# vineetbansal/scarlet

Measured on AMD Instinct MI355X. Metric: PGM iters/sec on 10k 5-band 64x64 scenes, higher is better.
Workload: dtype f32

## Files before the change

scarlet_amd/csrc/fused2.h:

```cpp
#pragma once
#include "fused.h"

#define SC_FB2 512
#define SC_NW2 (SC_FB2 / SC_WAVE)
#define SC_PAIR_VEC_FLOATS 512
__host__ __device__ inline size_t fused2_lds_bytes(int K, int H, int W)
{
    return sizeof(float) * ((size_t)K * H * tile_stride(W) + (size_t)K * SC_PAIR_VEC_FLOATS);
}
__host__ __device__ inline size_t fused2_exact_lds_bytes(int KM, int XS)
{
    return sizeof(float) * ((size_t)KM * XS * SC_XS_STRIDE + (size_t)KM * SC_PAIR_VEC_FLOATS);
}

struct KsLengths {
    unsigned short v[2][32];
    static constexpr int fast_len(int n)
    {
        for (int m = n;; ++m) {
            int q = m;
            while (q % 2 == 0) q /= 2;
            while (q % 3 == 0) q /= 3;
            while (q % 5 == 0) q /= 5;
            if (q == 1) return m;
        }
    }
    constexpr KsLengths() : v{}
    {
        for (int r = 0; r < 32; ++r) {
            const int F = fast_len(2 * (2 * r + 1) + 10);
            int Fe = F;
            while (Fe & 1) Fe = fast_len(Fe + 1);
            v[0][r] = (unsigned short)F; v[1][r] = (unsigned short)Fe;
        }
    }
};
__device__ const KsLengths sc_ks_lengths = KsLengths();
__device__ __forceinline__ unsigned ks_request_lengths(int tid)
{
    return tid < 64 ? (unsigned)(&sc_ks_lengths.v[0][0])[tid] : 0u;
}
__device__ __forceinline__ void ks_fill_lengths(unsigned short (*fl)[32], int tid, unsigned requested)
{
    if (tid < 64) (&fl[0][0])[tid] = (unsigned short)requested;
}
__device__ __forceinline__ KsGeom ks_geom(const SymWindow &s, const unsigned short (*fl)[32])
{
    KsGeom g;
    g.h = s.h; g.w = s.w; g.ry = s.h / 2; g.rx = s.w / 2;
    g.ntr = round16(s.h) >> 4; g.wp = round16(s.w); g.ntc = g.wp >> 4;
    g.Fy = uniform((int)fl[0][g.ry]);
    g.Fx = uniform((int)fl[1][g.rx]);
    return g;
}

template <int KM, int BM, int XS, bool P>
__device__ __forceinline__ int iterate2_body(const FusedArgs &a, const int s, const int c0, const int it_old, const bool resident,
                                             const bool reentered = false)
{
    static_assert(KM <= 4, "one pair of waves per component");
    static_assert(1 + KM * BM <= 32 && 4 * SC_NW2 == 32, "the partial sums are combined by 32 rows of 16 lanes");
    constexpr bool X = XS > 0;
    extern __shared__ __align__(16) float lds[];
    const int K = X ? KM : a.K, B = X ? BM : a.B, H = X ? XS : a.H, W = X ? XS : a.W, HW = H * W, LW = X ? SC_XS_STRIDE : tile_stride(W);
    const int tile_floats = H * LW;
#ifndef SC_TILE_B128
#define SC_TILE_B128 1
#endif
    auto tl4 = [](const float *p) {
        if constexpr (X && SC_TILE_B128 && (SC_XS_STRIDE % 4) == 0) return *reinterpret_cast<const float4 *>(p);
        else return lds_load4(p);
    };
    auto ts4 = [](float *p, float4 v) {
        if constexpr (X && SC_TILE_B128 && (SC_XS_STRIDE % 4) == 0) *reinterpret_cast<float4 *>(p) = v;
        else lds_store4(p, v);
    };
    const bool symmetric = X ? true : a.symmetric != 0, monotonic = X ? true : a.monotonic != 0;
    float *tiles = lds;
    float *vecs = lds + (size_t)K * tile_floats;
    constexpr int NG = KM * (KM + 1) / 2;
    constexpr int NP = 1 + KM * BM;
    constexpr int GPT = 2;
    constexpr int GPW = 8;
    __shared__ float red[4 * SC_NW2][NP > NG ? NP : NG];
    __shared__ double mat[2][KM * KM > BM * BM ? KM * KM : BM * BM];
    __shared__ float sed_s[KM * BM], sed_new[KM * BM];
    __shared__ float step_s[2];
    __shared__ double conv_s[KM][2], conv_m[KM][2][2];
    __shared__ int lstop_s[KM];
    __shared__ float nmax_s[KM][2];
    __shared__ int pair_flag[KM][2];
    __shared__ int arrive_s;
    __shared__ double cent_s[KM][2][3];
    __shared__ unsigned short fl_s[2][32];
    __shared__ int ctl_s[2][2];
    __shared__ int carry_cen[KM][2];
    __shared__ double carry_sh[KM][2];
    __shared__ float carry_sed[KM * BM];
    __shared__ short rowrange_s[KM][2][2];
    __shared__ unsigned place_s;
    const int tid = threadIdx.x, lane = tid & 63, wid = uniform(tid >> 6);
    float *const morph0 = a.morph[0], *const morph1 = a.morph[1], *const sed0 = a.sed[0], *const sed1 = a.sed[1];
    const float *min_g = (c0 ? morph1 : morph0) + (size_t)s * K * HW;
    float *mout_g = (c0 ? morph0 : morph1) + (size_t)s * K * HW;
    const float *sed_in = (c0 ? sed1 : sed0) + (size_t)s * K * B;
    float *sed_out = (c0 ? sed0 : sed1) + (size_t)s * K * B;
    const int it_new = it_old + 1;
    const int ngroups = HW >> 2, gpr = W >> 2;
    const float *img = a.images + (size_t)s * B * HW;
    const float *wgt = (!X && a.weights) ? a.weights + (size_t)s * B * HW : nullptr;
#define STAMP(i) do { if (a.stamps && tid == 0) a.stamps[(size_t)s * 16 + (i)] = (long long)__builtin_amdgcn_s_memtime(); } while (0)
#ifdef SC_STAMP_WORKER
#define WSTAMP(i) do { if (a.stamps && lane == 0) a.stamps[(size_t)s * 16 + 12 + (i)] = (long long)__builtin_amdgcn_s_memtime(); } while (0)
#else
#define WSTAMP(i) do { } while (0)
#endif
#ifdef SC_STAMP_PAIRS
    long long pst[3] = {0, 0, 0};
#define PSTAMP(i) do { if (a.stamps) pst[i] = (long long)__builtin_amdgcn_s_memtime(); } while (0)
#else
#define PSTAMP(i) do { } while (0)
#endif
    STAMP(0);
    if (a.stamps && tid == 0) a.stamps[(size_t)s * 16 + 7] = (long long)__builtin_amdgcn_s_memrealtime();
#ifdef SC_STAMP_PERIOD
    if (P && a.stamps && tid == 0) a.stamps[(size_t)a.S * 16 + (size_t)s * 2 + (it_new & 1)] = (long long)__builtin_amdgcn_s_memrealtime();
#endif
    if (P && a.stamps && tid == 0 && !reentered) {
        a.stamps[(size_t)s * 16 + 14] = (long long)__builtin_amdgcn_s_memrealtime();
        a.stamps[(size_t)s * 16 + 15] = (long long)__builtin_amdgcn_s_getreg(4 | (0 << 6) | (31 << 11))
                                        | ((long long)__builtin_amdgcn_s_getreg(20 | (0 << 6) | (31 << 11)) << 32);
    }
    const unsigned fl_req = ks_request_lengths(tid);
    const int n_present = a.ncomp ? scene_ncomp(a.ncomp, s, K) : K;
    const int slot = wid >> 1;
    int kp = slot;
    if constexpr (X) {
        unsigned place = 0x03020100u;
        if (P) { const unsigned lp = place_s; if (reentered) place = (unsigned)uniform((int)lp); }
        if (!(P && reentered) && !a.no_place) {
            int cost[KM];
#pragma unroll
            for (int j = 0; j < KM; ++j) {
                const int ccy = uniform(a.centers[2 * (s * K + j)]), ccx = uniform(a.centers[2 * (s * K + j) + 1]);
                const SymWindow w = sym_window(H, W, ccy, ccx);
                const int ntr = round16(w.h) >> 4, ntc = round16(w.w) >> 4;
                cost[j] = (j < n_present && !w.centered) ? ntr * ntc * (ntr + ntc) : 0;
            }
            place = 0;
#pragma unroll
            for (int j = 0; j < KM; ++j) {
                int rank = 0;
#pragma unroll
                for (int i = 0; i < KM; ++i) rank += (cost[i] > cost[j] || (cost[i] == cost[j] && i < j)) ? 1 : 0;
                place |= (unsigned)j << (8 * (rank ^ (rank >> 1)));
            }
        }
        if (P && !reentered && tid == 0) place_s = place;
        kp = (int)((place >> (8 * slot)) & (KM - 1));
    }
    int pre_cy = 0, pre_cx = 0;
    double pre_dy = 0, pre_dx = 0;
    if (X && kp < K) {
        const int cpre = s * K + kp;
        if (!(P && reentered)) {
            pre_cy = a.centers[2 * cpre]; pre_cx = a.centers[2 * cpre + 1];
            pre_dy = a.shifts[2 * cpre]; pre_dx = a.shifts[2 * cpre + 1];
        }
        if (P) {
            const int lcy = carry_cen[kp][0], lcx = carry_cen[kp][1];
            const double ldy = carry_sh[kp][0], ldx = carry_sh[kp][1];
            if (reentered) { pre_cy = lcy; pre_cx = lcx; pre_dy = ldy; pre_dx = ldx; }
        }
    }
    float *kcache = nullptr;
    float kc_v[3] = {0.f, 0.f, 0.f};
    unsigned kc_hdr = 0;
    if (X && a.kscache && kp < K) {
        kcache = a.kscache + ((size_t)(s * K + kp) * 2 + (wid & 1)) * SC_KSC_FLOATS;
        if (P) {
            kc_v[0] = __builtin_nontemporal_load(kcache + lane); kc_v[1] = __builtin_nontemporal_load(kcache + 64 + lane);
            kc_v[2] = __builtin_nontemporal_load(kcache + 128 + lane);
            kc_hdr = __builtin_nontemporal_load(reinterpret_cast<const unsigned *>(kcache) + 192 + (lane & 7));
        } else {
            kc_v[0] = kcache[lane]; kc_v[1] = kcache[64 + lane]; kc_v[2] = kcache[128 + lane];
            kc_hdr = reinterpret_cast<const unsigned *>(kcache)[192 + (lane & 7)];
        }
    }

    float4 mreg[GPT][KM];
    auto load4 = [&](const float *p, bool past_l1) {
        if (P && past_l1) {
            const f32x4 v = __builtin_nontemporal_load(reinterpret_cast<const f32x4 *>(p));
            return make_float4(v[0], v[1], v[2], v[3]);
        }
        return *reinterpret_cast<const float4 *>(p);
    };
    if (!P || !resident) {
#pragma unroll
        for (int j = 0; j < GPT; ++j) {
            const int g = tid + j * SC_FB2;
#pragma unroll
            for (int k = 0; k < KM; ++k)
                mreg[j][k] = (g < ngroups && k < K) ? load4(min_g + (size_t)k * HW + 4 * (size_t)g, reentered)
                                                   : make_float4(0.f, 0.f, 0.f, 0.f);
        }
    }
    float4 ireg[GPT][BM];
    auto load_images = [&](int j) {
        const int g = tid + j * SC_FB2;
#pragma unroll
        for (int b = 0; b < BM; ++b)
            ireg[j][b] = (g < ngroups && b < B) ? reinterpret_cast<const float4 *>(img + (size_t)b * HW)[g]
                                               : make_float4(0.f, 0.f, 0.f, 0.f);
    };
    load_images(0);
    for (int i = tid; i < K * B; i += SC_FB2) {
        float v = 0.f;
        if (!(P && reentered)) v = sed_in[i];
        if (P) { const float lv = carry_sed[(i / B) * BM + (i % B)]; if (reentered) v = lv; }
        if (P && !reentered) carry_sed[(i / B) * BM + (i % B)] = v;
        sed_s[(i / B) * BM + (i % B)] = v;
    }
    ks_fill_lengths(fl_s, tid, fl_req);
    if (tid < 2 * KM) (&pair_flag[0][0])[tid] = 0;
    if (tid == 2 * KM) arrive_s = 0;
    if (P && tid == 0) { ctl_s[it_old & 1][0] = 1; ctl_s[it_old & 1][1] = 1; }
    if (P && !reentered && tid < KM * 4) (&rowrange_s[0][0][0])[tid] = (short)((tid & 1) ? H - 1 : 0);
    if (P && resident) {
#pragma unroll
        for (int j = 0; j < GPT; ++j) {
            const int g = tid + j * SC_FB2;
            const int y = g / gpr, x = (g - y * gpr) << 2;
#pragma unroll
            for (int k = 0; k < KM; ++k)
                mreg[j][k] = (g < ngroups && k < K) ? tl4(tiles + k * tile_floats + y * LW + x) : make_float4(0.f, 0.f, 0.f, 0.f);
        }
    }
    const bool small_side = (K <= B);
    const bool carried = P && reentered && resident && monotonic && n_present > 0;
    auto sed_gram = [&](const float *sed, double *m) {
        double r = 0;
        if (small_side) {
            const int k = lane / K, k2 = lane - k * K;
            for (int b = 0; b < B; ++b) r += (double)sed[k * BM + b] * sed[k2 * BM + b];
            m[k * KM + k2] = r;
        } else {
            const int b = lane / B, b2 = lane - b * B;
            for (int k = 0; k < K; ++k) r += (double)sed[k * BM + b] * sed[k * BM + b2];
            m[b * BM + b2] = r;
        }
    };
    __syncthreads();
    {
        f32x2 gram2[NG];
#pragma unroll
        for (int i = 0; i < NG; ++i) gram2[i] = (f32x2){0.f, 0.f};
#pragma unroll
        for (int j = 0; j < GPT; ++j) {
            const int g = tid + j * SC_FB2;
            if (g < ngroups) {
                const int y = g / gpr, x = (g - y * gpr) << 2;
#pragma unroll
                for (int k = 0; k < KM; ++k)
                    if (k < K && !(P && resident)) ts4(tiles + k * tile_floats + y * LW + x, mreg[j][k]);
                int gi = 0;
#pragma unroll
                for (int k = 0; k < KM; ++k)
#pragma unroll
                    for (int k2 = k; k2 < KM; ++k2) {
                        const float4 p = mreg[j][k], q = mreg[j][k2];
                        gram2[gi] += (f32x2){p.x, p.y} * (f32x2){q.x, q.y};
                        gram2[gi] += (f32x2){p.z, p.w} * (f32x2){q.z, q.w};
                        ++gi;
                    }
            }
        }
        float gram[NG];
#pragma unroll
        for (int i = 0; i < NG; ++i) gram[i] = gram2[i].x + gram2[i].y;
        float gq[(NG + 3) / 4];
        wave_rowsum_quads(gram, gq);
        if ((lane & 12) == 12) {
#pragma unroll
            for (int m = 0; m < (NG + 3) / 4; ++m)
                if (4 * m + 3 < NG || 4 * m + (lane & 3) < NG) red[4 * wid + (lane >> 4)][4 * m + (lane & 3)] = gq[m];
        }
    }
#pragma unroll
    for (int j = 1; j < GPT; ++j) load_images(j);
    __syncthreads();
    STAMP(1);
    if (wid == 0) {
        {
            const int e = lane >> 2, q = lane & 3;
            const int k = e / K, k2 = e - k * K;
            const int lo = k < k2 ? k : k2, hi = k < k2 ? k2 : k;
            const int go = lo * KM - (lo * (lo - 1)) / 2 + (hi - lo);
            double r = 0;
            if (e < K * K) {
#pragma unroll
                for (int w = 0; w < SC_NW2; ++w) r += (double)red[q * SC_NW2 + w][go];
            }
            r += dpp_mov<SC_DPP_XOR1>(r);
            r += dpp_mov<SC_DPP_XOR2>(r);
            if (e < K * K && q == 0) mat[0][k * KM + k2] = r;
        }
        if (carried) {
            if (lane == 1) a.lipschitz[2 * s + 1] = mat[1][0];
        } else {
            if (lane < (small_side ? K * K : B * B)) sed_gram(sed_s, mat[1]);
            wave_sync();
            if (lane < 2 && !(monotonic && lane == 0)) {
                const int n = (lane == 0 || small_side) ? K : B, ld = (lane == 0 || small_side) ? KM : BM;
                const double L = n <= 4 ? lambda_max_charpoly4(mat[lane], n, ld) : jacobi_lambda_max(mat[lane], n, ld);
                step_s[lane] = 1.0f / (float)L;
                a.lipschitz[2 * s + lane] = L;
            }
        }
    }
    __syncthreads();
    STAMP(2);
    const float step_sed = step_s[0], step_morph = step_s[1];

    {
        float sed[KM][BM];
#pragma unroll
        for (int k = 0; k < KM; ++k)
#pragma unroll
            for (int b = 0; b < BM; ++b)
                sed[k][b] = (k < K && b < B) ? __builtin_bit_cast(float, __builtin_amdgcn_readfirstlane(
                                                   __builtin_bit_cast(int, sed_s[k * BM + b]))) : 0.f;
        bool fixm[KM];
#pragma unroll
        for (int k = 0; k < KM; ++k) fixm[k] = (k < K) && a.fix_morph && a.fix_morph[(size_t)s * K + k];
        f32x2 dsed2[KM][BM];
#pragma unroll
        for (int k = 0; k < KM; ++k)
#pragma unroll
            for (int b = 0; b < BM; ++b) dsed2[k][b] = (f32x2){0.f, 0.f};
        f32x2 loss2 = {0.f, 0.f};
        const f32x2 ws2 = {a.weight_scalar, a.weight_scalar};
#pragma unroll
        for (int j = 0; j < GPT; ++j) {
            const int g = tid + j * SC_FB2;
            if (g < ngroups) {
                const int y = g / gpr, x = (g - y * gpr) << 2;
                f32x2 m2[KM][2], gm2[KM][2];
#pragma unroll
                for (int k = 0; k < KM; ++k) {
                    float4 v = make_float4(0.f, 0.f, 0.f, 0.f);
                    if (k < K) v = tl4(tiles + k * tile_floats + y * LW + x);
                    m2[k][0] = (f32x2){v.x, v.y}; m2[k][1] = (f32x2){v.z, v.w};
                    gm2[k][0] = (f32x2){0.f, 0.f}; gm2[k][1] = gm2[k][0];
                }
#pragma unroll
                for (int b = 0; b < BM; ++b) {
                    if (b < B) {
                        const float4 iv = ireg[j][b];
                        f32x2 im2[2] = {{iv.x, iv.y}, {iv.z, iv.w}}, ww2[2] = {ws2, ws2};
                        if (wgt) {
                            const float4 wv = reinterpret_cast<const float4 *>(wgt + (size_t)b * HW)[g];
                            ww2[0] = (f32x2){wv.x, wv.y}; ww2[1] = (f32x2){wv.z, wv.w};
                        }
#pragma unroll
                        for (int p = 0; p < 2; ++p) {
                            f32x2 model = sed[0][b] * m2[0][p];
#pragma unroll
                            for (int k = 1; k < KM; ++k) model += sed[k][b] * m2[k][p];
                            const f32x2 d = X ? model - im2[p] : ww2[p] * (model - im2[p]);
                            loss2 = (f32x2){__builtin_fmaf(d.x, d.x, loss2.x), __builtin_fmaf(d.y, d.y, loss2.y)};
                            const f32x2 gg = X ? d : ww2[p] * d;
#pragma unroll
                            for (int k = 0; k < KM; ++k) { dsed2[k][b] += gg * m2[k][p]; gm2[k][p] += sed[k][b] * gg; }
                        }
                    }
                }
#pragma unroll
                for (int k = 0; k < KM; ++k)
                    if (k < K && !fixm[k]) {
                        const f32x2 o0 = m2[k][0] - step_morph * gm2[k][0], o1 = m2[k][1] - step_morph * gm2[k][1];
                        ts4(tiles + k * tile_floats + y * LW + x, make_float4(o0.x, o0.y, o1.x, o1.y));
                    }
            }
        }
        float part[NP];
        part[0] = 0.5f * (loss2.x + loss2.y);
#pragma unroll
        for (int k = 0; k < KM; ++k)
#pragma unroll
            for (int b = 0; b < BM; ++b) part[1 + k * BM + b] = dsed2[k][b].x + dsed2[k][b].y;
        float pq[(NP + 3) / 4];
        wave_rowsum_quads(part, pq);
        if ((lane & 12) == 12) {
#pragma unroll
            for (int m = 0; m < (NP + 3) / 4; ++m)
                if (4 * m + 3 < NP || 4 * m + (lane & 3) < NP) red[4 * wid + (lane >> 4)][4 * m + (lane & 3)] = pq[m];
        }
    }
    __syncthreads();
    STAMP(3);
    {
        const int i = tid >> 4, p = tid & 15;
        const bool live = i < 1 + K * B;
        const int src = (!live || i == 0) ? 0 : 1 + ((i - 1) / B) * BM + (i - 1) % B;
        double r = live ? (double)red[p][src] + (double)red[p + 16][src] : 0.0;
        r += dpp_mov<SC_DPP_XOR1>(r);
        r += dpp_mov<SC_DPP_XOR2>(r);
        r += dpp_mov<SC_DPP_HALF_MIRROR>(r);
        r += dpp_mov<SC_DPP_MIRROR>(r);
        if (live && p == 0) {
            if (i == 0) {
                if (it_new <= a.mse_capacity) a.mse[(size_t)s * a.mse_capacity + it_new - 1] = r;
            } else {
                const int k = (i - 1) / B, b = (i - 1) - k * B;
                if (monotonic) {
                    sed_new[k * BM + b] = (float)r;
                } else {
                    const float curv = sed_s[k * BM + b];
                    const bool fixed = a.fix_sed && a.fix_sed[(size_t)s * K + k];
                    sed_new[k * BM + b] = fixed ? curv : curv - step_sed * (float)r;
                }
            }
        }
    }
    __syncthreads();
    STAMP(4);

    const int k = kp, half = wid & 1;
    const bool lead = half == ((slot >> 1) & 1);
    auto pair_sync = [&](int phase, auto long_wait) {
        constexpr bool LONG = decltype(long_wait)::value;
        __builtin_amdgcn_fence(__ATOMIC_RELEASE, "workgroup");
        if (lane == 0) __hip_atomic_store(&pair_flag[k & (KM - 1)][half], phase, __ATOMIC_RELAXED, __HIP_MEMORY_SCOPE_WORKGROUP);
        while (__hip_atomic_load(&pair_flag[k & (KM - 1)][1 - half], __ATOMIC_RELAXED, __HIP_MEMORY_SCOPE_WORKGROUP) < phase) {
            if (LONG) __builtin_amdgcn_s_sleep(8); else __builtin_amdgcn_s_sleep(2);
        }
        __builtin_amdgcn_fence(__ATOMIC_ACQUIRE, "workgroup");
    };
    const bool mine = k < n_present;
    const int c = s * K + (mine ? k : 0);
    Tile t; t.H = H; t.W = W; t.LW = LW; t.m = tiles + (mine ? k : 0) * tile_floats;
    float *vec = vecs + (mine ? k : 0) * SC_PAIR_VEC_FLOATS;
    float *zv = vec + 384 + SC_WAVE * half;
    int cy = 0, cx = 0, stat = 0;
    int mode = 0;
    SymWindow sw = {0, 0, 1, 1, true};
    KsGeom kg = {};
    float sy = 0.f;
    bool rank1 = false;
    if (mine) {
        cy = X ? pre_cy : a.centers[2 * c]; cx = X ? pre_cx : a.centers[2 * c + 1];
        wave_max_pixel(t, cy, cx, stat);
        cy = uniform(cy); cx = uniform(cx);
        if (symmetric) {
            double dy = X ? pre_dy : a.shifts[2 * c], dx = X ? pre_dx : a.shifts[2 * c + 1];
            if (it_new % 5 == 0) {
                double p0, p1, p2;
                wave_centroid_sums(t, a.centroid_psf, a.centroid_P, cy, cx, half, 2, p0, p1, p2);
                if (lane == 0) { cent_s[k][half][0] = p0; cent_s[k][half][1] = p1; cent_s[k][half][2] = p2; }
                pair_sync(1, std::false_type{});
                wave_centroid_finish(t, a.centroid_P, cent_s[k][0][0] + cent_s[k][1][0], cent_s[k][0][1] + cent_s[k][1][1],
                                     cent_s[k][0][2] + cent_s[k][1][2], cy, cx, dy, dx, stat);
                if (lead && lane == 0) { a.shifts[2 * c] = dy; a.shifts[2 * c + 1] = dx; }
            }
            cy = uniform(cy); cx = uniform(cx); dy = uniform(dy); dx = uniform(dx);
            if (P && lead && lane == 0) { carry_cen[k][0] = cy; carry_cen[k][1] = cx; carry_sh[k][0] = dy; carry_sh[k][1] = dx; }
            sw = sym_window(H, W, cy, cx);
            mode = (dy != dy) ? 2 : (sw.centered ? 0 : 1);
            if (mode == 1) {
                kg = ks_geom(sw, fl_s);
                const unsigned key[6] = {(unsigned)H << 24 | (unsigned)W << 16 | (unsigned)cy << 8 | (unsigned)cx, SC_KSC_MAGIC,
                                         (unsigned)__double2loint(dy), (unsigned)__double2hiint(dy),
                                         (unsigned)__double2loint(dx), (unsigned)__double2hiint(dx)};
                bool hit = kcache != nullptr;
#pragma unroll
                for (int i = 0; i < 6; ++i) hit = hit && (unsigned)__builtin_amdgcn_readlane((int)kc_hdr, i) == key[i];
                if (hit) {
                    const int q = lane + SC_WAVE * half;
                    vec[q] = kc_v[0]; vec[128 + q] = kc_v[1]; vec[256 + q] = kc_v[2];
                    sy = __int_as_float(__builtin_amdgcn_readlane((int)kc_hdr, 6));
                } else {
                    sy = pair_ks_vectors(kg, dy, dx, vec, half, kc_v);
                    if (kcache) {
                        kcache[lane] = kc_v[0]; kcache[64 + lane] = kc_v[1]; kcache[128 + lane] = kc_v[2];
                        unsigned word = __float_as_uint(sy);
#pragma unroll
                        for (int i = 0; i < 6; ++i) word = lane == i ? key[i] : word;
                        if (lane < 7) reinterpret_cast<unsigned *>(kcache)[192 + lane] = word;
                    }
                }
                rank1 = sy != 0.f;
                if (rank1) pair_ks_colsums(t, sw, kg, zv);
            }
        }
    }
    STAMP(8);
    if (mine) pair_sync(2, std::false_type{});
#ifndef SC_STAMP_WORKER
    STAMP(12);
#endif
    f32x4 T[4][2];
    if (mine && mode == 1) {
        if (rank1) pair_ks_z(kg, vec + 256, zv);
        pair_ks_gemm1<true>(t, sw, kg, vec, half, T);
    }
    if (mine) pair_sync(3, std::false_type{});
#ifndef SC_STAMP_WORKER
    STAMP(13);
#endif
    if (mine && mode == 1) pair_ks_gemm2<true>(t, sw, kg, vec, zv, half, T, sy, rank1);
    if (mine && mode == 2 && lead) wave_flip_symmetry<float>(t, sw, false, 1.0f);
    if (mine) pair_sync(4, std::false_type{});
    STAMP(9);
    PSTAMP(0);
    const int dyq = (2 * SC_WAVE) / gpr, dxq = 2 * SC_WAVE - dyq * gpr;
    const int g0 = lane + SC_WAVE * half;
    const int y0 = g0 / gpr, x0 = g0 - y0 * gpr;
    int rl_lo = 0, rl_hi = H - 1, ro_lo = 0, ro_hi = H - 1;
    if (P && mine) {
        rl_lo = uniform((int)rowrange_s[k][c0][0]); rl_hi = uniform((int)rowrange_s[k][c0][1]);
        ro_lo = uniform((int)rowrange_s[k][1 - c0][0]); ro_hi = uniform((int)rowrange_s[k][1 - c0][1]);
    }
    float4 lastv[GPW];
    auto load_last = [&]() {
        const float4 *last4 = reinterpret_cast<const float4 *>(min_g + (size_t)k * HW);
#pragma unroll
        for (int j = 0; j < GPW; ++j) {
            const int g = g0 + j * 2 * SC_WAVE;
            const int row = y0 + j * dyq;
            const bool want = g < ngroups && (!P || (row >= rl_lo && row <= rl_hi));
            lastv[j] = want ? load4(reinterpret_cast<const float *>(last4 + g), true) : make_float4(0.f, 0.f, 0.f, 0.f);
        }
    };
    float l0 = (!X && a.l0_thresh >= 0.f) ? a.l0_thresh * step_morph : -1.f;
    float l1 = (!X && a.l1_thresh >= 0.f) ? a.l1_thresh * step_morph : -1.f;
    auto sparse = [&](float v) {
        if (l0 >= 0.f && fabsf(v) < l0) v = 0.f;
        if (l1 >= 0.f) {
            const float mag = fabsf(v) - l1;
            v = (v > 0.f ? 1.f : (v < 0.f ? -1.f : 0.f)) * (mag < 0.f ? 0.f : mag);
        }
        return v;
    };
    if (mine && !lead) load_last();
    if (monotonic && mine && !lead) {
        float peak = sparse(t.m[cy * LW + cx]);
        if (peak < 0.f) peak = 0.f;
        int arrived = 0;
        if (lane == 0) nmax_s[k][1] = peak;
        __builtin_amdgcn_fence(__ATOMIC_RELEASE, "workgroup");
        if (lane == 0) arrived = __hip_atomic_fetch_add(&arrive_s, 1, __ATOMIC_RELAXED, __HIP_MEMORY_SCOPE_WORKGROUP);
        if (uniform(arrived) == n_present - 1) {
            __builtin_amdgcn_fence(__ATOMIC_ACQUIRE, "workgroup");
            WSTAMP(0);
            float step_w = 0.f;
            if (lane == 0) {
                const double L = lambda_max_charpoly4(mat[0], K, KM);
                a.lipschitz[2 * s] = L;
                step_w = 1.0f / (float)L;
            }
            step_w = read_lane(step_w, 0);
            const int kk = lane >> 4, bb = lane & 15;
            const bool entry = kk < n_present && bb < B;
            double d2s = 0, n2s = 0;
            if (entry) {
                const float curv = sed_s[kk * BM + bb];
                const bool fixed = a.fix_sed && a.fix_sed[(size_t)s * K + kk];
                float v = fixed ? curv : curv - step_w * sed_new[kk * BM + bb];
                if (v < 0.f) v = 0.f;
                v = v * nmax_s[kk][1];
                sed_out[kk * B + bb] = v;
                if (P) carry_sed[kk * BM + bb] = v;
                const float d = curv - v;
                d2s = (double)(d * d);
                n2s = (double)(v * v);
            }
            d2s = row_sum(d2s); n2s = row_sum(n2s);
            if (entry && bb == 0) { conv_s[kk][0] = d2s; conv_s[kk][1] = n2s; }
            if (P) {
                wave_sync();
                if (lane < (small_side ? K * K : B * B)) sed_gram(carry_sed, mat[1]);
                wave_sync();
                if (lane == 0) {
                    const int n = small_side ? K : B, ld = small_side ? KM : BM;
                    const double L = n <= 4 ? lambda_max_charpoly4(mat[1], n, ld) : jacobi_lambda_max(mat[1], n, ld);
                    step_s[1] = 1.0f / (float)L;
                    mat[1][0] = L;
                }
            }
            WSTAMP(1);
        }
    }
    if (mine && lead) {
        int lstop = 1 << 30;
        if (monotonic) wave_monotonic<float>(t, cy, cx, 0.f, &lstop);
        if (lane == 0) {
            lstop_s[k] = lstop; a.centers[2 * c] = cy; a.centers[2 * c + 1] = cx;
            if (P) nmax_s[k][0] = t.m[cy * LW + cx];
        }
        load_last();
    }
    if (mine) pair_sync(5, std::true_type{});
    STAMP(10);
    PSTAMP(1);
    float norm = 0.f;
    if (!monotonic) {
        float vmax = -INFINITY;
        bool anynan = false;
        if (mine) {
            int y = y0, xq = x0;
            for (int g = g0; g < ngroups; g += 2 * SC_WAVE) {
                float *p = t.m + y * LW + (xq << 2);
                float4 v = lds_load4(p);
                v.x = sparse(v.x); v.y = sparse(v.y); v.z = sparse(v.z); v.w = sparse(v.w);
                v.x = v.x < 0.f ? 0.f : v.x; v.y = v.y < 0.f ? 0.f : v.y;
                v.z = v.z < 0.f ? 0.f : v.z; v.w = v.w < 0.f ? 0.f : v.w;
                anynan |= (v.x != v.x) | (v.y != v.y) | (v.z != v.z) | (v.w != v.w);
                vmax = fmaxf(fmaxf(vmax, fmaxf(v.x, v.y)), fmaxf(v.z, v.w));
                lds_store4(p, v);
                y += dyq; xq += dxq;
                if (xq >= gpr) { xq -= gpr; ++y; }
            }
            vmax = wave_max(vmax);
            if (__any(anynan)) vmax = __builtin_nanf("");
            if (lane == 0) nmax_s[k][half] = vmax;
        }
        if (mine) pair_sync(6, std::false_type{});
        if (mine) {
            const float m0 = nmax_s[k][0], m1 = nmax_s[k][1];
            norm = (m0 != m0 || m1 != m1) ? __builtin_nanf("") : fmaxf(m0, m1);
        }
        l0 = -1.f; l1 = -1.f;
    } else if (mine) {
        norm = sparse(P ? nmax_s[k][0] : t.m[cy * LW + cx]);
        if (norm < 0.f) norm = 0.f;
    }
    if (mine) {
        const int lstop = lstop_s[k];
        const bool cut = lstop < (1 << 30);
        const bool regular = norm > 0.f && !isinf(norm);
        const float rnorm = 1.0f / norm;
        float4 *out4 = reinterpret_cast<float4 *>(mout_g + (size_t)k * HW);
        f32x2 d2p = {0.f, 0.f}, n2p = {0.f, 0.f};
        const f32x2 rn2 = {rnorm, rnorm}, nm2 = {norm, norm};
        int u_lo = 0, u_hi = H - 1;
        if (P && cut && regular && l0 < 0.f && l1 < 0.f) {
            const int rt = lstop >> 1;
            u_lo = min(min(rl_lo, ro_lo), max(cy - rt, 0)); u_hi = max(max(rl_hi, ro_hi), min(cy + rt, H - 1));
        }
        auto final_pass = [&](auto cut_c, auto gen_c) {
            constexpr bool CUT = decltype(cut_c)::value, GEN = decltype(gen_c)::value;
            int y = y0, xq = x0;
#pragma unroll
            for (int j = 0; j < GPW; ++j) {
                const int g = g0 + j * 2 * SC_WAVE;
                const int yw = uniform(y0 + j * dyq) & ~3;
                const bool skip = P && X && (yw + 3 < u_lo || yw > u_hi);
                if (g < ngroups && skip) ts4(t.m + y * LW + (xq << 2), make_float4(0.f, 0.f, 0.f, 0.f));
                if (g < ngroups && !skip) {
                    const float4 v4 = tl4(t.m + y * LW + (xq << 2));
                    const float4 l = lastv[j];
                    float v[4] = {v4.x, v4.y, v4.z, v4.w};
                    int axmax = 0, xb = 0;
                    if (CUT) {
                        const int ay = y < cy ? cy - y : y - cy;
                        const int h1 = (lstop - ay) >> 1;
                        axmax = h1 >= ay ? h1 : lstop - 2 * ay;
                        xb = (xq << 2) - cx + axmax;
                    }
#pragma unroll
                    for (int e = 0; e < 4; ++e) {
                        if (GEN) v[e] = sparse(v[e]);
                        const bool beyond = CUT && (axmax < 0 || (unsigned)(xb + e) > (unsigned)(2 * axmax));
                        v[e] = (v[e] < 0.f || beyond) ? 0.f : v[e];
                    }
                    f32x2 o01, o23;
                    if (GEN && !regular) {
                        o01 = (f32x2){v[0] / norm, v[1] / norm}; o23 = (f32x2){v[2] / norm, v[3] / norm};
                    } else {
                        const f32x2 a01 = {v[0], v[1]}, a23 = {v[2], v[3]};
                        const f32x2 q01 = a01 * rn2, q23 = a23 * rn2;
                        o01 = (a01 - q01 * nm2) * rn2 + q01;
                        o23 = (a23 - q23 * nm2) * rn2 + q23;
                    }
                    const float4 o4 = make_float4(o01.x, o01.y, o23.x, o23.y);
                    out4[g] = o4;
                    if (P) ts4(t.m + y * LW + (xq << 2), o4);
                    const f32x2 e01 = (f32x2){l.x, l.y} - o01, e23 = (f32x2){l.z, l.w} - o23;
                    d2p += e01 * e01; d2p += e23 * e23;
                    n2p += o01 * o01; n2p += o23 * o23;
                }
                y += dyq; xq += dxq;
                if (xq >= gpr) { xq -= gpr; ++y; }
                if (j & 1) __builtin_amdgcn_sched_barrier(0);
            }
        };
        using std::true_type; using std::false_type;
        if (regular && l0 < 0.f && l1 < 0.f) {
            if (cut) final_pass(true_type{}, false_type{}); else final_pass(false_type{}, false_type{});
        } else {
            final_pass(true_type{}, true_type{});
        }
        const double d2 = wave_sum((double)(d2p.x + d2p.y)), n2 = wave_sum((double)(n2p.x + n2p.y));
        if (lane == 0) { conv_m[k][half][0] = d2; conv_m[k][half][1] = n2; }
        if (P && lead && lane == 0) {
            const bool known = cut && regular && l0 < 0.f && l1 < 0.f;
            rowrange_s[k][1 - c0][0] = (short)(known ? max(cy - (lstop >> 1), 0) : 0);
            rowrange_s[k][1 - c0][1] = (short)(known ? min(cy + (lstop >> 1), H - 1) : H - 1);
        }
        if (lead && !monotonic) {
            double d2s = 0, n2s = 0;
            if (lane < B) {
                float v = sed_new[k * BM + lane];
                if (v < 0.f) v = 0.f;
                v = v * norm;
                sed_out[k * B + lane] = v;
                if (P) carry_sed[k * BM + lane] = v;
                const float d = sed_s[k * BM + lane] - v;
                d2s = (double)(d * d);
                n2s = (double)(v * v);
            }
            d2s = wave_sum(d2s); n2s = wave_sum(n2s);
            if (lane == 0) { conv_s[k][0] = d2s; conv_s[k][1] = n2s; }
        }
    }
#ifdef SC_STAMP_PAIRS
    PSTAMP(2);
    if (a.stamps && mine && lead && lane == 0) {
        long long *q = a.stamps + (size_t)a.S * 16 + (size_t)s * 8 + 2 * k;
        const int ls = lstop_s[k];
        q[0] = pst[2];
        q[1] = ((pst[2] - pst[1]) & 0xfffff) | (((pst[1] - pst[0]) & 0xfffff) << 20) | ((long long)(ls < 255 ? ls : 255) << 40) |
               ((long long)kg.ntr << 48) | ((long long)kg.ntc << 51) | ((long long)slot << 54);
    }
#endif
    __syncthreads();
    if (mine && norm == norm) {
        const double n2 = conv_m[k][0][1] + conv_m[k][1][1];
        if (n2 != n2) {
            norm = __builtin_nanf("");
            float4 *out4 = reinterpret_cast<float4 *>(mout_g + (size_t)k * HW);
            const float4 nan4 = make_float4(norm, norm, norm, norm);
            for (int g = g0; g < ngroups; g += 2 * SC_WAVE) out4[g] = nan4;
            if (lead && lane < B) { sed_out[k * B + lane] = norm; if (P) carry_sed[k * BM + lane] = norm; }
            if (P && lane == 0) {
                ctl_s[it_old & 1][1] = 0;
                rowrange_s[k][1 - c0][0] = 0; rowrange_s[k][1 - c0][1] = (short)(H - 1);
            }
        }
    }
    if (mine && lead && lane == 0) {
        if (!(norm > 0.f) || isinf(norm)) stat |= SCARLET_STATUS_NONFINITE;
        if (stat) atomicOr(&a.status[s], stat);
    }
    STAMP(5);

    if (wid == 0) {
        bool pending = false;
        if (lane < n_present && it_new > 1) {
            const int kk = lane;
            int set = 0;
            const double d2 = conv_m[kk][0][0] + conv_m[kk][1][0], n2 = conv_m[kk][0][1] + conv_m[kk][1][1];
            if (!(n2 == n2 && conv_s[kk][0] <= a.e_rel2 * conv_s[kk][1])) set |= SCARLET_FLAG_SED_NOT_CONVERGED;
            if (!(d2 <= a.e_rel2 * n2)) set |= SCARLET_FLAG_MORPH_NOT_CONVERGED;
            const int clear = (SCARLET_FLAG_SED_NOT_CONVERGED | SCARLET_FLAG_MORPH_NOT_CONVERGED) & ~set;
            if (clear) atomicAnd(&a.flags[s * K + kk], ~clear);
            if (set) atomicOr(&a.flags[s * K + kk], set);
            pending = set != 0;
        }
        const bool done = it_new > 1 && __builtin_amdgcn_ballot_w64(pending) == 0;
        if (lane == 0) {
            a.it[s] = it_new;
            a.cur[s] = 1 - c0;
            if (done) { a.active[s] = 0; if (P) ctl_s[it_old & 1][0] = 0; }
        }
    }
    STAMP(6);
    if (a.stamps && tid == 0) a.stamps[(size_t)s * 16 + 11] = (long long)__builtin_amdgcn_s_memrealtime();
#undef STAMP
#undef WSTAMP
#undef PSTAMP
    if (P) {
        __syncthreads();
        return uniform(ctl_s[it_old & 1][0] | (ctl_s[it_old & 1][1] << 1));
    }
    return 0;
}

template <int KM, int BM, int XS = 0>
__global__ __launch_bounds__(SC_FB2, 4) void k_iterate2(FusedArgs a)
{
    const int s = blockIdx.x;
    const int active_s = a.active[s], c0 = a.cur[s], it_old = a.it[s];
    asm volatile("" ::"s"(c0), "s"(it_old));
    if (!active_s) return;
    iterate2_body<KM, BM, XS, false>(a, s, c0, it_old, false);
}

#define SC_FIT2X_KERNEL k_fit2x
#define SC_FIT2X_REENTER(scene, state, it)                                                                     \
    asm volatile("s_mov_b64 exec, -1\n\t"                                                                      \
                 "s_mov_b64 s[0:1], %0\n\t"                                                                    \
                 "s_mov_b32 s2, %1\n\t"                                                                        \
                 "s_mov_b32 s3, %2\n\t"                                                                        \
                 "s_mov_b32 s4, %3\n\t"                                                                        \
                 "v_mov_b32 v0, %4\n\t"                                                                        \
                 "s_getpc_b64 s[6:7]\n\t"                                                                      \
                 "s_add_u32 s6, s6, k_fit2x@rel32@lo+4\n\t"                                                    \
                 "s_addc_u32 s7, s7, k_fit2x@rel32@hi+12\n\t"                                                  \
                 "s_waitcnt lgkmcnt(0)\n\t"                                                                    \
                 "s_setpc_b64 s[6:7]"                                                                          \
                 :                                                                                             \
                 : "s"(__builtin_amdgcn_kernarg_segment_ptr()), "s"(scene), "s"(state), "s"(it), "v"((int)threadIdx.x) \
                 : "s0", "s1", "s2", "s3", "s4", "s6", "s7", "v0", "scc", "memory")
extern "C" __global__ __launch_bounds__(SC_FB2, 4) void SC_FIT2X_KERNEL(FusedArgs a, int n_iter, int *queue, int n_workgroups)
{
    const int s = blockIdx.x;
    const unsigned st = (unsigned)__builtin_amdgcn_workgroup_id_y();
    int c0 = 0, it = 0, left = 0;
    bool resident = false, run = true;
    if (st >> 31) {
        resident = ((st >> 30) & 1) && !(n_iter & (1 << 30));
        c0 = (int)((st >> 29) & 1); left = (int)(st & 0x1fffffffu);
        it = (int)__builtin_amdgcn_workgroup_id_z();
    } else {
        const int active_s = a.active[s];
        c0 = a.cur[s]; it = a.it[s];
        asm volatile("" ::"s"(c0), "s"(it));
        left = n_iter & 0xffffff;
        run = active_s && left > 0;
    }
    if (run) {
        const int r = iterate2_body<4, 5, 64, true>(a, s, c0, it, resident, (st >> 31) != 0);
        if ((r & 1) && left > 1) {
            const unsigned nst = 0x80000000u | ((unsigned)(r >> 1) << 30) | ((unsigned)(c0 ^ 1) << 29) | (unsigned)(left - 1);
            if (!(r & 2) || (n_iter & (1 << 30))) {
                asm volatile("s_waitcnt vmcnt(0)" ::: "memory");
                __syncthreads();
            }
            SC_FIT2X_REENTER(s, nst, it + 1);
        }
    }
    __shared__ int next_s;
    if (threadIdx.x == 0) next_s = queue ? atomicAdd(queue, 1) + n_workgroups : a.S;
    __syncthreads();
    const int nx = uniform(next_s);
    __syncthreads();
    if (nx < a.S) SC_FIT2X_REENTER(nx, 0u, 0);
}
```

Before: 16.60 million.

## Add fast prologue path for reentered resident iterations, skipping redundant setup

Wraps the per-iteration prologue in a lambda instantiated twice, so a specialized FAST variant runs when the persistent kernel re-enters with morph data still resident. That variant reads placement, centers, shifts and SEDs only from LDS carry state and skips the FFT length requests and global loads. It drops the barrier before the Gram computation and caches n_present inside place_s. The Gram accumulation also uses explicit FMAs. The cost is doubled code size for the prologue and some extra register pressure.

```diff
diff --git a/scarlet_amd/csrc/fused2.h b/scarlet_amd/csrc/fused2.h
--- a/scarlet_amd/csrc/fused2.h
+++ b/scarlet_amd/csrc/fused2.h
@@ -100,6 +100,7 @@
     __shared__ short rowrange_s[KM][2][2];
     __shared__ unsigned place_s;
     const int tid = threadIdx.x, lane = tid & 63, wid = uniform(tid >> 6);
+    if constexpr (X) __builtin_assume(tid >= 0 && tid < SC_FB2);
     float *const morph0 = a.morph[0], *const morph1 = a.morph[1], *const sed0 = a.sed[0], *const sed1 = a.sed[1];
     const float *min_g = (c0 ? morph1 : morph0) + (size_t)s * K * HW;
     float *mout_g = (c0 ? morph0 : morph1) + (size_t)s * K * HW;
@@ -121,24 +122,60 @@
 #else
 #define PSTAMP(i) do { } while (0)
 #endif
+#ifdef SC_STAMP_PROLOGUE
+#define QSTAMP(i) STAMP(12 + (i))
+#else
+#define QSTAMP(i) do { } while (0)
+#endif
+    int n_present = K;
+    if (X && a.ncomp && !(P && reentered)) n_present = scene_ncomp(a.ncomp, s, K);
     STAMP(0);
     if (a.stamps && tid == 0) a.stamps[(size_t)s * 16 + 7] = (long long)__builtin_amdgcn_s_memrealtime();
 #ifdef SC_STAMP_PERIOD
     if (P && a.stamps && tid == 0) a.stamps[(size_t)a.S * 16 + (size_t)s * 2 + (it_new & 1)] = (long long)__builtin_amdgcn_s_memrealtime();
 #endif
     if (P && a.stamps && tid == 0 && !reentered) {
+#ifndef SC_STAMP_PROLOGUE
         a.stamps[(size_t)s * 16 + 14] = (long long)__builtin_amdgcn_s_memrealtime();
+#endif
         a.stamps[(size_t)s * 16 + 15] = (long long)__builtin_amdgcn_s_getreg(4 | (0 << 6) | (31 << 11))
                                         | ((long long)__builtin_amdgcn_s_getreg(20 | (0 << 6) | (31 << 11)) << 32);
     }
-    const unsigned fl_req = ks_request_lengths(tid);
-    const int n_present = a.ncomp ? scene_ncomp(a.ncomp, s, K) : K;
     const int slot = wid >> 1;
     int kp = slot;
+    int pre_cy = 0, pre_cx = 0;
+    double pre_dy = 0, pre_dx = 0;
+    float *kcache = nullptr;
+    float kc_v[3] = {0.f, 0.f, 0.f};
+    unsigned kc_hdr = 0;
+    float4 ireg[GPT][BM];
+    auto load_images = [&](int j) {
+        const int g = tid + j * SC_FB2;
+#pragma unroll
+        for (int b = 0; b < BM; ++b)
+            ireg[j][b] = (g < ngroups && b < B) ? reinterpret_cast<const float4 *>(img + (size_t)b * HW)[g]
+                                               : make_float4(0.f, 0.f, 0.f, 0.f);
+    };
+    auto load4 = [&](const float *p, bool past_l1) {
+        if (P && past_l1) {
+            const f32x4 v = __builtin_nontemporal_load(reinterpret_cast<const f32x4 *>(p));
+            return make_float4(v[0], v[1], v[2], v[3]);
+        }
+        return *reinterpret_cast<const float4 *>(p);
+    };
+    auto phase0 = [&](auto fast_c) {
+    constexpr bool FAST = P && decltype(fast_c)::value;
+    const bool reent = FAST || reentered, resid = FAST || resident;
+    if (FAST) load_images(0);
+    const unsigned fl_req = (P && reent) ? 0u : ks_request_lengths(tid);
+    if (!X && a.ncomp) n_present = scene_ncomp(a.ncomp, s, K);
     if constexpr (X) {
         unsigned place = 0x03020100u;
-        if (P) { const unsigned lp = place_s; if (reentered) place = (unsigned)uniform((int)lp); }
-        if (!(P && reentered) && !a.no_place) {
+        if (FAST) {
+            place = (unsigned)uniform((int)place_s);
+        } else if (P) { const unsigned lp = place_s; if (reent) place = (unsigned)uniform((int)lp); }
+        if (P && reent && a.ncomp) n_present = (int)((place >> 4) & 7u);
+        if (!(P && reent) && !a.no_place) {
             int cost[KM];
 #pragma unroll
             for (int j = 0; j < KM; ++j) {
@@ -156,26 +193,26 @@
                 place |= (unsigned)j << (8 * (rank ^ (rank >> 1)));
             }
         }
-        if (P && !reentered && tid == 0) place_s = place;
+        if (P && !reent && tid == 0) place_s = place | ((unsigned)n_present << 4);
         kp = (int)((place >> (8 * slot)) & (KM - 1));
     }
-    int pre_cy = 0, pre_cx = 0;
-    double pre_dy = 0, pre_dx = 0;
     if (X && kp < K) {
         const int cpre = s * K + kp;
-        if (!(P && reentered)) {
-            pre_cy = a.centers[2 * cpre]; pre_cx = a.centers[2 * cpre + 1];
-            pre_dy = a.shifts[2 * cpre]; pre_dx = a.shifts[2 * cpre + 1];
-        }
-        if (P) {
-            const int lcy = carry_cen[kp][0], lcx = carry_cen[kp][1];
-            const double ldy = carry_sh[kp][0], ldx = carry_sh[kp][1];
-            if (reentered) { pre_cy = lcy; pre_cx = lcx; pre_dy = ldy; pre_dx = ldx; }
-        }
-    }
-    float *kcache = nullptr;
-    float kc_v[3] = {0.f, 0.f, 0.f};
-    unsigned kc_hdr = 0;
+        if (FAST) {
+            pre_cy = carry_cen[kp][0]; pre_cx = carry_cen[kp][1];
+            pre_dy = carry_sh[kp][0]; pre_dx = carry_sh[kp][1];
+        } else {
+            if (!(P && reent)) {
+                pre_cy = a.centers[2 * cpre]; pre_cx = a.centers[2 * cpre + 1];
+                pre_dy = a.shifts[2 * cpre]; pre_dx = a.shifts[2 * cpre + 1];
+            }
+            if (P) {
+                const int lcy = carry_cen[kp][0], lcx = carry_cen[kp][1];
+                const double ldy = carry_sh[kp][0], ldx = carry_sh[kp][1];
+                if (reent) { pre_cy = lcy; pre_cx = lcx; pre_dy = ldy; pre_dx = ldx; }
+            }
+        }
+    }
     if (X && a.kscache && kp < K) {
         kcache = a.kscache + ((size_t)(s * K + kp) * 2 + (wid & 1)) * SC_KSC_FLOATS;
         if (P) {
@@ -189,45 +226,35 @@
     }
 
     float4 mreg[GPT][KM];
-    auto load4 = [&](const float *p, bool past_l1) {
-        if (P && past_l1) {
-            const f32x4 v = __builtin_nontemporal_load(reinterpret_cast<const f32x4 *>(p));
-            return make_float4(v[0], v[1], v[2], v[3]);
-        }
-        return *reinterpret_cast<const float4 *>(p);
-    };
-    if (!P || !resident) {
+    if (!P || !resid) {
 #pragma unroll
         for (int j = 0; j < GPT; ++j) {
             const int g = tid + j * SC_FB2;
 #pragma unroll
             for (int k = 0; k < KM; ++k)
-                mreg[j][k] = (g < ngroups && k < K) ? load4(min_g + (size_t)k * HW + 4 * (size_t)g, reentered)
+                mreg[j][k] = (g < ngroups && k < K) ? load4(min_g + (size_t)k * HW + 4 * (size_t)g, reent)
                                                    : make_float4(0.f, 0.f, 0.f, 0.f);
         }
     }
-    float4 ireg[GPT][BM];
-    auto load_images = [&](int j) {
-        const int g = tid + j * SC_FB2;
-#pragma unroll
-        for (int b = 0; b < BM; ++b)
-            ireg[j][b] = (g < ngroups && b < B) ? reinterpret_cast<const float4 *>(img + (size_t)b * HW)[g]
-                                               : make_float4(0.f, 0.f, 0.f, 0.f);
-    };
-    load_images(0);
+    if (!FAST) load_images(0);
     for (int i = tid; i < K * B; i += SC_FB2) {
         float v = 0.f;
-        if (!(P && reentered)) v = sed_in[i];
-        if (P) { const float lv = carry_sed[(i / B) * BM + (i % B)]; if (reentered) v = lv; }
-        if (P && !reentered) carry_sed[(i / B) * BM + (i % B)] = v;
+        if (FAST) {
+            v = carry_sed[(i / B) * BM + (i % B)];
+        } else {
+            if (!(P && reent)) v = sed_in[i];
+            if (P) { const float lv = carry_sed[(i / B) * BM + (i % B)]; if (reent) v = lv; }
+        }
+        if (P && !reent) carry_sed[(i / B) * BM + (i % B)] = v;
         sed_s[(i / B) * BM + (i % B)] = v;
     }
-    ks_fill_lengths(fl_s, tid, fl_req);
+    QSTAMP(0);
+    if (!(P && reent)) ks_fill_lengths(fl_s, tid, fl_req);
     if (tid < 2 * KM) (&pair_flag[0][0])[tid] = 0;
     if (tid == 2 * KM) arrive_s = 0;
     if (P && tid == 0) { ctl_s[it_old & 1][0] = 1; ctl_s[it_old & 1][1] = 1; }
-    if (P && !reentered && tid < KM * 4) (&rowrange_s[0][0][0])[tid] = (short)((tid & 1) ? H - 1 : 0);
-    if (P && resident) {
+    if (P && !reent && tid < KM * 4) (&rowrange_s[0][0][0])[tid] = (short)((tid & 1) ? H - 1 : 0);
+    if (P && resid) {
 #pragma unroll
         for (int j = 0; j < GPT; ++j) {
             const int g = tid + j * SC_FB2;
@@ -237,6 +264,51 @@
                 mreg[j][k] = (g < ngroups && k < K) ? tl4(tiles + k * tile_floats + y * LW + x) : make_float4(0.f, 0.f, 0.f, 0.f);
         }
     }
+    if (!FAST) __syncthreads();
+    QSTAMP(1);
+    {
+        f32x2 gram2[NG];
+#pragma unroll
+        for (int i = 0; i < NG; ++i) gram2[i] = (f32x2){0.f, 0.f};
+#pragma unroll
+        for (int j = 0; j < GPT; ++j) {
+            const int g = tid + j * SC_FB2;
+            if (g < ngroups) {
+                const int y = g / gpr, x = (g - y * gpr) << 2;
+#pragma unroll
+                for (int k = 0; k < KM; ++k)
+                    if (k < K && !(P && resid)) ts4(tiles + k * tile_floats + y * LW + x, mreg[j][k]);
+                int gi = 0;
+#pragma unroll
+                for (int k = 0; k < KM; ++k)
+#pragma unroll
+                    for (int k2 = k; k2 < KM; ++k2) {
+                        const float4 p = mreg[j][k], q = mreg[j][k2];
+                        const f32x2 pl = {p.x, p.y}, ph = {p.z, p.w}, ql = {q.x, q.y}, qh = {q.z, q.w};
+                        if (j == 0 && k2 == k) {
+                            gram2[gi] = __builtin_elementwise_fma(pl, ql, ph * qh);
+                        } else {
+                            gram2[gi] = __builtin_elementwise_fma(pl, ql, gram2[gi]);
+                            gram2[gi] = __builtin_elementwise_fma(ph, qh, gram2[gi]);
+                        }
+                        ++gi;
+                    }
+            }
+        }
+        float gram[NG];
+#pragma unroll
+        for (int i = 0; i < NG; ++i) gram[i] = gram2[i].x + gram2[i].y;
+        float gq[(NG + 3) / 4];
+        wave_rowsum_quads(gram, gq);
+        if ((lane & 12) == 12) {
+#pragma unroll
+            for (int m = 0; m < (NG + 3) / 4; ++m)
+                if (4 * m + 3 < NG || 4 * m + (lane & 3) < NG) red[4 * wid + (lane >> 4)][4 * m + (lane & 3)] = gq[m];
+        }
+    }
+    };
+    if (P && reentered && resident) phase0(std::true_type{}); else phase0(std::false_type{});
+    if (P) { kp = uniform(kp); n_present = uniform(n_present); }
     const bool small_side = (K <= B);
     const bool carried = P && reentered && resident && monotonic && n_present > 0;
     auto sed_gram = [&](const float *sed, double *m) {
@@ -251,42 +323,6 @@
             m[b * BM + b2] = r;
         }
     };
-    __syncthreads();
-    {
-        f32x2 gram2[NG];
-#pragma unroll
-        for (int i = 0; i < NG; ++i) gram2[i] = (f32x2){0.f, 0.f};
-#pragma unroll
-        for (int j = 0; j < GPT; ++j) {
-            const int g = tid + j * SC_FB2;
-            if (g < ngroups) {
-                const int y = g / gpr, x = (g - y * gpr) << 2;
-#pragma unroll
-                for (int k = 0; k < KM; ++k)
-                    if (k < K && !(P && resident)) ts4(tiles + k * tile_floats + y * LW + x, mreg[j][k]);
-                int gi = 0;
-#pragma unroll
-                for (int k = 0; k < KM; ++k)
-#pragma unroll
-                    for (int k2 = k; k2 < KM; ++k2) {
-                        const float4 p = mreg[j][k], q = mreg[j][k2];
-                        gram2[gi] += (f32x2){p.x, p.y} * (f32x2){q.x, q.y};
-                        gram2[gi] += (f32x2){p.z, p.w} * (f32x2){q.z, q.w};
-                        ++gi;
-                    }
-            }
-        }
-        float gram[NG];
-#pragma unroll
-        for (int i = 0; i < NG; ++i) gram[i] = gram2[i].x + gram2[i].y;
-        float gq[(NG + 3) / 4];
-        wave_rowsum_quads(gram, gq);
-        if ((lane & 12) == 12) {
-#pragma unroll
-            for (int m = 0; m < (NG + 3) / 4; ++m)
-                if (4 * m + 3 < NG || 4 * m + (lane & 3) < NG) red[4 * wid + (lane >> 4)][4 * m + (lane & 3)] = gq[m];
-        }
-    }
 #pragma unroll
     for (int j = 1; j < GPT; ++j) load_images(j);
     __syncthreads();
@@ -354,6 +390,7 @@
                     m2[k][0] = (f32x2){v.x, v.y}; m2[k][1] = (f32x2){v.z, v.w};
                     gm2[k][0] = (f32x2){0.f, 0.f}; gm2[k][1] = gm2[k][0];
                 }
+                if (j == 0) QSTAMP(2);
 #pragma unroll
                 for (int b = 0; b < BM; ++b) {
                     if (b < B) {
@@ -497,7 +534,7 @@
     }
     STAMP(8);
     if (mine) pair_sync(2, std::false_type{});
-#ifndef SC_STAMP_WORKER
+#if !defined(SC_STAMP_WORKER) && !defined(SC_STAMP_PROLOGUE)
     STAMP(12);
 #endif
     f32x4 T[4][2];
@@ -506,7 +543,7 @@
         pair_ks_gemm1<true>(t, sw, kg, vec, half, T);
     }
     if (mine) pair_sync(3, std::false_type{});
-#ifndef SC_STAMP_WORKER
+#if !defined(SC_STAMP_WORKER) && !defined(SC_STAMP_PROLOGUE)
     STAMP(13);
 #endif
     if (mine && mode == 1) pair_ks_gemm2<true>(t, sw, kg, vec, zv, half, T, sy, rank1);
@@ -779,6 +816,7 @@
     STAMP(6);
     if (a.stamps && tid == 0) a.stamps[(size_t)s * 16 + 11] = (long long)__builtin_amdgcn_s_memrealtime();
 #undef STAMP
+#undef QSTAMP
 #undef WSTAMP
 #undef PSTAMP
     if (P) {
@@ -818,6 +856,7 @@
 {
     const int s = blockIdx.x;
     const unsigned st = (unsigned)__builtin_amdgcn_workgroup_id_y();
+    asm volatile("" ::"s"(a.images), "s"(a.stamps), "s"(a.ncomp));
     int c0 = 0, it = 0, left = 0;
     bool resident = false, run = true;
     if (st >> 31) {
```

Measured after the change: 17.05 million (median of 6 runs). 2.7% higher.
